# omerbt/TokenFlow

Hardware: NVIDIA H100
Metric: frames/sec for 40-frame 512x512 SD1.5 50-step edit (higher is better)
Workload: dtype fp16

## Files before the change

### tokenflow_b200/csrc/tf_common.cuh

```cuda
#pragma once

#include <cuda.h>
#include <cuda_fp16.h>
#include <cuda_runtime.h>
#include <stdint.h>
#include <stdio.h>

namespace tf {

void set_last_error(const char* fmt, ...);
int  check_cuda(cudaError_t e, const char* what);

enum Status : int {
  TF_OK = 0,
  TF_ERR_INVALID_ARGUMENT = 1,
  TF_ERR_CUDA = 2,
  TF_ERR_UNSUPPORTED = 3,
  TF_ERR_DRIVER = 4,
};

CUresult encode_tiled(CUtensorMap* map, CUtensorMapDataType dtype, uint32_t rank, const void* base,
                      const uint64_t* dims, const uint64_t* strides_bytes ,
                      const uint32_t* box, CUtensorMapSwizzle swizzle);

int sm_count();

#ifdef __CUDACC__
__device__ __forceinline__ uint32_t smem_u32(const void* p) {
  return static_cast<uint32_t>(__cvta_generic_to_shared(p));
}
__device__ __forceinline__ uint32_t lane_id() { return threadIdx.x & 31u; }

__device__ __forceinline__ void mbar_init(uint64_t* bar, uint32_t count) {
  asm volatile("mbarrier.init.shared::cta.b64 [%0], %1;" ::"r"(smem_u32(bar)), "r"(count) : "memory");
}
__device__ __forceinline__ void fence_mbar_init() {
  asm volatile("fence.mbarrier_init.release.cluster;" ::: "memory");
}
__device__ __forceinline__ void mbar_arrive(uint64_t* bar) {
  asm volatile("mbarrier.arrive.shared::cta.b64 _, [%0];" ::"r"(smem_u32(bar)) : "memory");
}
__device__ __forceinline__ void mbar_arrive_expect_tx(uint64_t* bar, uint32_t bytes) {
  asm volatile("mbarrier.arrive.expect_tx.shared::cta.b64 _, [%0], %1;" ::"r"(smem_u32(bar)), "r"(bytes)
               : "memory");
}
__device__ __forceinline__ bool mbar_try_wait(uint64_t* bar, uint32_t parity) {
  uint32_t ok;
  asm volatile(
      "{\n\t.reg .pred p;\n\t"
      "mbarrier.try_wait.parity.shared::cta.b64 p, [%1], %2;\n\t"
      "selp.u32 %0, 1, 0, p;\n\t}\n"
      : "=r"(ok)
      : "r"(smem_u32(bar)), "r"(parity)
      : "memory");
  return ok != 0;
}
__device__ __forceinline__ uint64_t global_timer_ns() {
  uint64_t t;
  asm volatile("mov.u64 %0, %%globaltimer;" : "=l"(t));
  return t;
}
__device__ __forceinline__ void mbar_wait(uint64_t* bar, uint32_t parity) {
  uint32_t spins = 0;
  uint64_t t0 = 0;
  while (!mbar_try_wait(bar, parity)) {
    if ((++spins & 2047u) == 0) {
      const uint64_t now = global_timer_ns();
      if (t0 == 0) t0 = now;
      if (now - t0 > 2000000000ull) __trap();
    }
  }
}

__device__ __forceinline__ void tma_prefetch_desc(const CUtensorMap* m) {
  asm volatile("prefetch.tensormap [%0];" ::"l"(reinterpret_cast<uint64_t>(m)) : "memory");
}
__device__ __forceinline__ void tma_load_3d(void* smem_dst, const CUtensorMap* m, uint64_t* bar, int c0,
                                            int c1, int c2) {
  asm volatile(
      "cp.async.bulk.tensor.3d.shared::cluster.global.tile.mbarrier::complete_tx::bytes"
      " [%0], [%1, {%3, %4, %5}], [%2];"
      ::"r"(smem_u32(smem_dst)), "l"(reinterpret_cast<uint64_t>(m)), "r"(smem_u32(bar)), "r"(c0), "r"(c1),
      "r"(c2)
      : "memory");
}
__device__ __forceinline__ void tma_load_4d(void* smem_dst, const CUtensorMap* m, uint64_t* bar, int c0,
                                            int c1, int c2, int c3) {
  asm volatile(
      "cp.async.bulk.tensor.4d.shared::cluster.global.tile.mbarrier::complete_tx::bytes"
      " [%0], [%1, {%3, %4, %5, %6}], [%2];"
      ::"r"(smem_u32(smem_dst)), "l"(reinterpret_cast<uint64_t>(m)), "r"(smem_u32(bar)), "r"(c0), "r"(c1),
      "r"(c2), "r"(c3)
      : "memory");
}

__device__ __forceinline__ uint64_t wgmma_desc(uint32_t smem_addr, uint32_t lbo_bytes, uint32_t sbo_bytes) {
  uint64_t d = 0;
  d |= static_cast<uint64_t>((smem_addr & 0x3FFFFu) >> 4);
  d |= static_cast<uint64_t>((lbo_bytes >> 4) & 0x3FFFu) << 16;
  d |= static_cast<uint64_t>((sbo_bytes >> 4) & 0x3FFFu) << 32;
  d |= static_cast<uint64_t>(1) << 62;
  return d;
}
__device__ __forceinline__ void wgmma_fence() { asm volatile("wgmma.fence.sync.aligned;" ::: "memory"); }
__device__ __forceinline__ void wgmma_commit() { asm volatile("wgmma.commit_group.sync.aligned;" ::: "memory"); }
template <int kPending>
__device__ __forceinline__ void wgmma_wait() {
  asm volatile("wgmma.wait_group.sync.aligned %0;" ::"n"(kPending) : "memory");
}
template <int N>
__device__ __forceinline__ void reg_fence(float (&r)[N]) {
#pragma unroll
  for (int i = 0; i < N; ++i) asm volatile("" : "+f"(r[i])::"memory");
}

__device__ __forceinline__ uint32_t pack_f16x2_rn(float lo, float hi) {
  uint32_t r;
  asm("cvt.rn.f16x2.f32 %0, %1, %2;" : "=r"(r) : "f"(hi), "f"(lo));
  return r;
}
__device__ __forceinline__ float fast_exp2(float x) {
  float y;
  asm("ex2.approx.ftz.f32 %0, %1;" : "=f"(y) : "f"(x));
  return y;
}
#endif

}
```

### tokenflow_b200/csrc/tf_ext_attn.cu

```cuda
#include <cmath>
#include <type_traits>

#include "tf_common.cuh"
#include "tf_kernels.h"
#include "tf_wgmma.cuh"

namespace tf {
namespace {

constexpr int kBlockM = 128;
constexpr int kMaxStages = 8;
constexpr int kSmemBudget = 227 * 1024;

struct AttnCtl {
  uint64_t q_full;
  uint64_t full[kMaxStages];
  uint64_t empty[kMaxStages];
};

struct AttnParams {
  int S, heads, d;
  int tiles_m;
  int stages;
  float scale_log2;
  long long out_tok_stride;
  int q_row0;
  int q_row_end;
  int out_rows;
};

struct Item {
  int out_u, out_c, q, k0, v_u0, v_c0, n_kv;
};
__device__ __forceinline__ Item item_of(const AttnTable& t, int i) {
  const AttnSample& s = t.s[i];
  return {s.out_sample, -1, s.q_sample, s.k_sample0, s.v_sample0, -1, s.n_kv};
}
__device__ __forceinline__ Item item_of(const AttnPairTable& t, int i) {
  const AttnPair& p = t.p[i];
  return {p.out_u, p.out_c, p.q_sample, p.k_sample0, p.v_u0, p.v_c0, p.n_kv};
}

template <int kDChunks, int kBlockN, int kNPV, class Tab>
__global__ void __launch_bounds__(256, 1)
ext_attn_kernel(const __grid_constant__ CUtensorMap map_q, const __grid_constant__ CUtensorMap map_k,
                const __grid_constant__ CUtensorMap map_v, const __grid_constant__ Tab tab, const AttnParams prm,
                __half* __restrict__ out) {
  constexpr int kNV = std::is_same<Tab, AttnPairTable>::value ? 2 : 1;
  constexpr int kQChunkBytes = kBlockM * 128;
  constexpr int kKVChunkBytes = kBlockN * 128;
  constexpr int kQBytes = kDChunks * kQChunkBytes;
  constexpr int kTileBytes = kDChunks * kKVChunkBytes;
  constexpr int kStageBytes = (1 + kNV) * kTileBytes;
  constexpr int kS = kBlockN / 2;
  constexpr int kO = kNPV / 2;
  static_assert(kNPV <= 64 * kDChunks, "P V width exceeds the loaded channels");

  extern __shared__ uint8_t smem_raw[];
  uint8_t* smem = reinterpret_cast<uint8_t*>((reinterpret_cast<uintptr_t>(smem_raw) + 1023) & ~uintptr_t(1023));
  uint8_t* q_smem = smem;
  uint8_t* ring = smem + kQBytes;
  AttnCtl* ctl = reinterpret_cast<AttnCtl*>(ring + prm.stages * kStageBytes);

  const int S = prm.S, d = prm.d, stages = prm.stages;
  const int per_sample = prm.heads * prm.tiles_m;
  const int slot = blockIdx.x / per_sample;
  const int rem = blockIdx.x - slot * per_sample;
  const int head = rem / prm.tiles_m;
  const int m0 = prm.q_row0 + (rem - head * prm.tiles_m) * kBlockM;
  const Item it = item_of(tab, slot);
  const int tiles_per_slab = (S + kBlockN - 1) / kBlockN;
  const int T = it.n_kv * tiles_per_slab;
  const int ksteps = (d + 15) / 16;

  auto load_tile = [&](int t) {
    const int st = t % stages;
    const int slab = t / tiles_per_slab;
    const int n0 = (t - slab * tiles_per_slab) * kBlockN;
    uint8_t* dst = ring + st * kStageBytes;
    mbar_arrive_expect_tx(&ctl->full[st], (uint32_t)kStageBytes);
#pragma unroll
    for (int c = 0; c < kDChunks; ++c) {
      tma_load_4d(dst + c * kKVChunkBytes, &map_k, &ctl->full[st], c * 64, head, n0, it.k0 + slab);
      tma_load_4d(dst + kTileBytes + c * kKVChunkBytes, &map_v, &ctl->full[st], c * 64, head, n0, it.v_u0 + slab);
      if (kNV == 2)
        tma_load_4d(dst + 2 * kTileBytes + c * kKVChunkBytes, &map_v, &ctl->full[st], c * 64, head, n0,
                    it.v_c0 + slab);
    }
  };

  if (threadIdx.x == 0) {
    tma_prefetch_desc(&map_q);
    tma_prefetch_desc(&map_k);
    tma_prefetch_desc(&map_v);
    mbar_init(&ctl->q_full, 1);
    for (int i = 0; i < stages; ++i) {
      mbar_init(&ctl->full[i], 1);
      mbar_init(&ctl->empty[i], 8);
    }
    fence_mbar_init();
  }
  __syncthreads();
  if (threadIdx.x == 0) {
    mbar_arrive_expect_tx(&ctl->q_full, (uint32_t)kQBytes);
#pragma unroll
    for (int c = 0; c < kDChunks; ++c) tma_load_4d(q_smem + c * kQChunkBytes, &map_q, &ctl->q_full, c * 64, head, m0, it.q);
    for (int t = 0; t < stages && t < T; ++t) load_tile(t);
  }
  __syncwarp();

  const int wg = threadIdx.x >> 7;
  const int lane = threadIdx.x & 31;
  const int wrow = ((threadIdx.x >> 5) & 3) * 16 + (lane >> 2);
  const int qcol = 2 * (lane & 3);

  float o[kNV][kO];
#pragma unroll
  for (int v = 0; v < kNV; ++v)
#pragma unroll
    for (int i = 0; i < kO; ++i) o[v][i] = 0.f;
  float m_r[2] = {-INFINITY, -INFINITY}, l_r[2] = {0.f, 0.f};
  const float sl2 = prm.scale_log2;

  const uint32_t q_addr = smem_u32(q_smem) + wg * 64 * 128;
  const uint32_t ring_addr = smem_u32(ring);
  mbar_wait(&ctl->q_full, 0);
  __syncwarp();

  for (int t = 0; t < T; ++t) {
    const int st = t % stages;
    mbar_wait(&ctl->full[st], (uint32_t)(t / stages) & 1u);
    __syncwarp();
    const uint32_t k_addr = ring_addr + st * kStageBytes;

    float s[kS];
    wgmma_fence();
    for (int kk = 0; kk < ksteps; ++kk) {
      const uint32_t off = (kk & 3) * 32;
      wgmma_ss<kBlockN>(s, wgmma_desc(q_addr + (kk >> 2) * kQChunkBytes + off, 16, 1024),
                        wgmma_desc(k_addr + (kk >> 2) * kKVChunkBytes + off, 16, 1024), kk > 0 ? 1u : 0u);
    }
    wgmma_commit();
    wgmma_wait<0>();
    reg_fence(s);

    const int n0 = (t % tiles_per_slab) * kBlockN;
    if (n0 + kBlockN > S) {
      const int valid = S - n0;
#pragma unroll
      for (int j = 0; j < kBlockN / 8; ++j) {
        const int c = 8 * j + qcol;
        if (c >= valid) { s[4 * j] = -INFINITY; s[4 * j + 2] = -INFINITY; }
        if (c + 1 >= valid) { s[4 * j + 1] = -INFINITY; s[4 * j + 3] = -INFINITY; }
      }
    }

    float mx[2] = {-INFINITY, -INFINITY};
#pragma unroll
    for (int j = 0; j < kBlockN / 8; ++j) {
      mx[0] = fmaxf(mx[0], fmaxf(s[4 * j], s[4 * j + 1]));
      mx[1] = fmaxf(mx[1], fmaxf(s[4 * j + 2], s[4 * j + 3]));
    }
    float corr[2], mneg[2];
#pragma unroll
    for (int r = 0; r < 2; ++r) {
      mx[r] = fmaxf(mx[r], __shfl_xor_sync(0xffffffffu, mx[r], 1));
      mx[r] = fmaxf(mx[r], __shfl_xor_sync(0xffffffffu, mx[r], 2));
      const float m_new = fmaxf(m_r[r], mx[r] * sl2);
      corr[r] = fast_exp2(m_r[r] - m_new);
      m_r[r] = m_new;
      mneg[r] = -m_new;
      l_r[r] *= corr[r];
    }
    uint32_t pa[kBlockN / 16][4];
#pragma unroll
    for (int j = 0; j < kBlockN / 8; ++j) {
      const float p0 = fast_exp2(fmaf(s[4 * j], sl2, mneg[0]));
      const float p1 = fast_exp2(fmaf(s[4 * j + 1], sl2, mneg[0]));
      const float p2 = fast_exp2(fmaf(s[4 * j + 2], sl2, mneg[1]));
      const float p3 = fast_exp2(fmaf(s[4 * j + 3], sl2, mneg[1]));
      l_r[0] += p0 + p1;
      l_r[1] += p2 + p3;
      pa[j >> 1][(j & 1) * 2 + 0] = pack_f16x2_rn(p0, p1);
      pa[j >> 1][(j & 1) * 2 + 1] = pack_f16x2_rn(p2, p3);
    }
#pragma unroll
    for (int v = 0; v < kNV; ++v)
#pragma unroll
      for (int j = 0; j < kO / 4; ++j) {
        o[v][4 * j] *= corr[0]; o[v][4 * j + 1] *= corr[0];
        o[v][4 * j + 2] *= corr[1]; o[v][4 * j + 3] *= corr[1];
      }

#pragma unroll
    for (int v = 0; v < kNV; ++v) reg_fence(o[v]);
    wgmma_fence();
#pragma unroll
    for (int kk = 0; kk < kBlockN / 16; ++kk)
#pragma unroll
      for (int v = 0; v < kNV; ++v)
        wgmma_rs<kNPV>(o[v], pa[kk], wgmma_desc(k_addr + (1 + v) * kTileBytes + kk * 16 * 128, kKVChunkBytes, 1024), 1u);
    wgmma_commit();
    wgmma_wait<0>();
#pragma unroll
    for (int v = 0; v < kNV; ++v) reg_fence(o[v]);

    __syncwarp();
    if (lane == 0) mbar_arrive(&ctl->empty[st]);
    if (threadIdx.x == 0 && t >= 1 && t - 1 + stages < T) {
      const int pt = t - 1;
      mbar_wait(&ctl->empty[pt % stages], (uint32_t)(pt / stages) & 1u);
      load_tile(pt + stages);
    }
    __syncwarp();
  }

#pragma unroll
  for (int r = 0; r < 2; ++r) {
    l_r[r] += __shfl_xor_sync(0xffffffffu, l_r[r], 1);
    l_r[r] += __shfl_xor_sync(0xffffffffu, l_r[r], 2);
    l_r[r] = 1.f / l_r[r];
  }
#pragma unroll
  for (int v = 0; v < kNV; ++v) {
    const int out_slab = v == 0 ? it.out_u : it.out_c;
#pragma unroll
    for (int r = 0; r < 2; ++r) {
      const int tok = m0 + wg * 64 + wrow + 8 * r;
      if (tok >= prm.q_row_end) continue;
      __half* dst = out + ((long long)out_slab * prm.out_rows + (tok - prm.q_row0)) * prm.out_tok_stride + head * d;
#pragma unroll
      for (int j = 0; j < kO / 4; ++j) {
        const int c = 8 * j + qcol;
        if (c < d)
          *reinterpret_cast<uint32_t*>(dst + c) = pack_f16x2_rn(o[v][4 * j + 2 * r] * l_r[r], o[v][4 * j + 2 * r + 1] * l_r[r]);
      }
    }
  }
}

template <int kDChunks, int kBlockN, int kNPV, class Tab>
int launch_cfg(const void* q, const void* k, const void* v, long long q_tok_stride, long long kv_tok_stride,
               int q_samples_total, int kv_samples_total, const Tab& tab, int n_items, int S, int heads, int d,
               float scale, void* out, int q_row0, int q_nrows, cudaStream_t stream) {
  constexpr int kNV = std::is_same<Tab, AttnPairTable>::value ? 2 : 1;
  constexpr int kQBytes = kDChunks * kBlockM * 128;
  constexpr int kStageBytes = (1 + kNV) * kDChunks * kBlockN * 128;
  int stages = (kSmemBudget - 2048 - kQBytes) / kStageBytes;
  if (stages > kMaxStages) stages = kMaxStages;
  if (stages < 2) { set_last_error("tf_ext_attn: configuration does not fit shared memory"); return TF_ERR_UNSUPPORTED; }
  const size_t smem_bytes = 1024 + kQBytes + (size_t)stages * kStageBytes + sizeof(AttnCtl);

  CUtensorMap map_q, map_k, map_v;
  auto make = [&](CUtensorMap* m, const void* base, long long tok_stride, int samples, int box_rows) -> int {
    const uint64_t dims[4] = {(uint64_t)d, (uint64_t)heads, (uint64_t)S, (uint64_t)samples};
    const uint64_t strides[3] = {(uint64_t)d * 2, (uint64_t)tok_stride * 2, (uint64_t)S * tok_stride * 2};
    const uint32_t box[4] = {64, 1, (uint32_t)box_rows, 1};
    CUresult r = encode_tiled(m, CU_TENSOR_MAP_DATA_TYPE_FLOAT16, 4, base, dims, strides, box,
                              CU_TENSOR_MAP_SWIZZLE_128B);
    if (r != CUDA_SUCCESS) { set_last_error("tf_ext_attn: cuTensorMapEncodeTiled failed: %d", (int)r); return TF_ERR_DRIVER; }
    return TF_OK;
  };
  if (int e = make(&map_q, q, q_tok_stride, q_samples_total, kBlockM)) return e;
  if (int e = make(&map_k, k, kv_tok_stride, kv_samples_total, kBlockN)) return e;
  if (int e = make(&map_v, v, kv_tok_stride, kv_samples_total, kBlockN)) return e;

  AttnParams prm;
  prm.S = S; prm.heads = heads; prm.d = d;
  prm.q_row0 = q_row0; prm.q_row_end = (q_row0 + q_nrows < S) ? q_row0 + q_nrows : S; prm.out_rows = q_nrows;
  prm.tiles_m = (prm.q_row_end - q_row0 + kBlockM - 1) / kBlockM;
  prm.stages = stages;
  prm.scale_log2 = scale * 1.4426950408889634f;
  prm.out_tok_stride = (long long)heads * d;

  auto kern = ext_attn_kernel<kDChunks, kBlockN, kNPV, Tab>;
  if (check_cuda(cudaFuncSetAttribute(kern, cudaFuncAttributeMaxDynamicSharedMemorySize, (int)smem_bytes),
                 "tf_ext_attn smem attribute"))
    return TF_ERR_CUDA;
  const long long grid = (long long)n_items * heads * prm.tiles_m;
  kern<<<(unsigned)grid, 256, smem_bytes, stream>>>(map_q, map_k, map_v, tab, prm, static_cast<__half*>(out));
  return check_cuda(cudaGetLastError(), "tf_ext_attn launch");
}

template <class Tab>
int dispatch(const void* q, const void* k, const void* v, long long q_tok_stride, long long kv_tok_stride,
             int q_samples_total, int kv_samples_total, const Tab& tab, int n_items, int S, int heads, int d,
             float scale, void* out, int q_row0, int q_nrows, cudaStream_t stream) {
  constexpr bool kPair = std::is_same<Tab, AttnPairTable>::value;
#define TF_CFG(C, N, P)                                                                                          \
  case P:                                                                                                       \
    if constexpr (!kPair || P <= 64)                                                                            \
      return launch_cfg<C, N, P, Tab>(q, k, v, q_tok_stride, kv_tok_stride, q_samples_total, kv_samples_total,  \
                                      tab, n_items, S, heads, d, scale, out, q_row0, q_nrows, stream);          \
    break
  switch ((d + 15) / 16 * 16) {
    TF_CFG(1, 128, 16); TF_CFG(1, 128, 32); TF_CFG(1, 128, 48); TF_CFG(1, 128, 64);
    TF_CFG(2, 128, 80); TF_CFG(2, 128, 96); TF_CFG(2, 128, 112); TF_CFG(2, 128, 128);
    TF_CFG(3, 64, 144); TF_CFG(3, 64, 160); TF_CFG(3, 64, 176); TF_CFG(3, 64, 192);
    default: break;
  }
#undef TF_CFG
  set_last_error("tf_ext_attn: head dim %d > 192 is not supported", d);
  return TF_ERR_UNSUPPORTED;
}

}

int launch_ext_attn(const void* q, const void* k, const void* v, long long q_tok_stride, long long kv_tok_stride,
                    int q_samples_total, int kv_samples_total, const AttnTable& tab, int n_out, int S, int heads,
                    int d, float scale, void* out, int q_row0, int q_nrows, cudaStream_t stream) {
  if (n_out == 0 || S == 0 || q_nrows <= 0 || q_row0 >= S) return TF_OK;
  return dispatch(q, k, v, q_tok_stride, kv_tok_stride, q_samples_total, kv_samples_total, tab, n_out, S, heads, d,
                  scale, out, q_row0, q_nrows, stream);
}

bool ext_attn_pairs_supported(int d) {
  return d <= 64;
}

int launch_ext_attn_pairs(const void* q, const void* k, const void* v, long long q_tok_stride, long long kv_tok_stride,
                          int q_samples_total, int kv_samples_total, const AttnPairTable& tab, int n_pairs, int S,
                          int heads, int d, float scale, void* out, int q_row0, int q_nrows, cudaStream_t stream) {
  if (n_pairs == 0 || S == 0 || q_nrows <= 0 || q_row0 >= S) return TF_OK;
  if (!ext_attn_pairs_supported(d)) {
    set_last_error("tf_ext_attn: paired kernel does not cover d=%d", d);
    return TF_ERR_UNSUPPORTED;
  }
  return dispatch(q, k, v, q_tok_stride, kv_tok_stride, q_samples_total, kv_samples_total, tab, n_pairs, S, heads, d,
                  scale, out, q_row0, q_nrows, stream);
}

}
```

Before: 2.886.

## Overlap QK and PV wgmma across iterations with ping-pong warpgroup scheduling

Restructures the extended-attention main loop so the QK^T wgmma for tile t is issued together with the PV wgmma for tile t-1, and softmax runs while PV is in flight. Named barriers make the two warpgroups take turns issuing tensor-core work, in the style of FlashAttention-3. The empty mbarriers are replaced by a shared atomic counter, and the last warp to release a stage issues its refill. This adds register pressure (s and pa are live across iterations) and more complex synchronization, which risks spills or ordering bugs in the barrier and atomic refill path.

```diff
diff --git a/tokenflow_b200/csrc/tf_common.cuh b/tokenflow_b200/csrc/tf_common.cuh
--- a/tokenflow_b200/csrc/tf_common.cuh
+++ b/tokenflow_b200/csrc/tf_common.cuh
@@ -72,6 +72,13 @@
   }
 }
 
+__device__ __forceinline__ void named_bar_sync(uint32_t id, uint32_t count) {
+  asm volatile("bar.sync %0, %1;" ::"r"(id), "r"(count) : "memory");
+}
+__device__ __forceinline__ void named_bar_arrive(uint32_t id, uint32_t count) {
+  asm volatile("bar.arrive %0, %1;" ::"r"(id), "r"(count) : "memory");
+}
+
 __device__ __forceinline__ void tma_prefetch_desc(const CUtensorMap* m) {
   asm volatile("prefetch.tensormap [%0];" ::"l"(reinterpret_cast<uint64_t>(m)) : "memory");
 }
diff --git a/tokenflow_b200/csrc/tf_ext_attn.cu b/tokenflow_b200/csrc/tf_ext_attn.cu
--- a/tokenflow_b200/csrc/tf_ext_attn.cu
+++ b/tokenflow_b200/csrc/tf_ext_attn.cu
@@ -15,7 +15,7 @@
 struct AttnCtl {
   uint64_t q_full;
   uint64_t full[kMaxStages];
-  uint64_t empty[kMaxStages];
+  uint32_t released[kMaxStages];
 };
 
 struct AttnParams {
@@ -41,8 +41,32 @@
   return {p.out_u, p.out_c, p.q_sample, p.k_sample0, p.v_u0, p.v_c0, p.n_kv};
 }
 
+constexpr int kThreads = 256;
+constexpr int kWarps = kThreads / 32;
+constexpr uint32_t kTurnBar = 1;
+
+template <int kBlockN, int kNPV, int kQChunkBytes, int kKVChunkBytes>
+__device__ __forceinline__ void issue_qk(float (&s)[kBlockN / 2], uint32_t q_addr, uint32_t k_addr) {
+#pragma unroll
+  for (int kk = 0; kk < kNPV / 16; ++kk) {
+    const uint32_t off = (kk & 3) * 32;
+    wgmma_ss<kBlockN>(s, wgmma_desc(q_addr + (kk >> 2) * kQChunkBytes + off, 16, 1024),
+                      wgmma_desc(k_addr + (kk >> 2) * kKVChunkBytes + off, 16, 1024), kk > 0 ? 1u : 0u);
+  }
+}
+
+template <int kBlockN, int kNPV, int kNV, int kTileBytes, int kKVChunkBytes>
+__device__ __forceinline__ void issue_pv(float (&o)[kNV][kNPV / 2], const uint32_t (&pa)[kBlockN / 16][4],
+                                         uint32_t k_addr) {
+#pragma unroll
+  for (int kk = 0; kk < kBlockN / 16; ++kk)
+#pragma unroll
+    for (int v = 0; v < kNV; ++v)
+      wgmma_rs<kNPV>(o[v], pa[kk], wgmma_desc(k_addr + (1 + v) * kTileBytes + kk * 16 * 128, kKVChunkBytes, 1024), 1u);
+}
+
 template <int kDChunks, int kBlockN, int kNPV, class Tab>
-__global__ void __launch_bounds__(256, 1)
+__global__ void __launch_bounds__(kThreads, 1)
 ext_attn_kernel(const __grid_constant__ CUtensorMap map_q, const __grid_constant__ CUtensorMap map_k,
                 const __grid_constant__ CUtensorMap map_v, const __grid_constant__ Tab tab, const AttnParams prm,
                 __half* __restrict__ out) {
@@ -71,20 +95,19 @@
   const Item it = item_of(tab, slot);
   const int tiles_per_slab = (S + kBlockN - 1) / kBlockN;
   const int T = it.n_kv * tiles_per_slab;
-  const int ksteps = (d + 15) / 16;
 
   auto load_tile = [&](int t) {
-    const int st = t % stages;
+    const int stage = t % stages;
     const int slab = t / tiles_per_slab;
-    const int n0 = (t - slab * tiles_per_slab) * kBlockN;
-    uint8_t* dst = ring + st * kStageBytes;
-    mbar_arrive_expect_tx(&ctl->full[st], (uint32_t)kStageBytes);
+    const int kn0 = (t - slab * tiles_per_slab) * kBlockN;
+    uint8_t* dst = ring + stage * kStageBytes;
+    mbar_arrive_expect_tx(&ctl->full[stage], (uint32_t)kStageBytes);
 #pragma unroll
     for (int c = 0; c < kDChunks; ++c) {
-      tma_load_4d(dst + c * kKVChunkBytes, &map_k, &ctl->full[st], c * 64, head, n0, it.k0 + slab);
-      tma_load_4d(dst + kTileBytes + c * kKVChunkBytes, &map_v, &ctl->full[st], c * 64, head, n0, it.v_u0 + slab);
+      tma_load_4d(dst + c * kKVChunkBytes, &map_k, &ctl->full[stage], c * 64, head, kn0, it.k0 + slab);
+      tma_load_4d(dst + kTileBytes + c * kKVChunkBytes, &map_v, &ctl->full[stage], c * 64, head, kn0, it.v_u0 + slab);
       if (kNV == 2)
-        tma_load_4d(dst + 2 * kTileBytes + c * kKVChunkBytes, &map_v, &ctl->full[st], c * 64, head, n0,
+        tma_load_4d(dst + 2 * kTileBytes + c * kKVChunkBytes, &map_v, &ctl->full[stage], c * 64, head, kn0,
                     it.v_c0 + slab);
     }
   };
@@ -96,7 +119,7 @@
     mbar_init(&ctl->q_full, 1);
     for (int i = 0; i < stages; ++i) {
       mbar_init(&ctl->full[i], 1);
-      mbar_init(&ctl->empty[i], 8);
+      ctl->released[i] = 0;
     }
     fence_mbar_init();
   }
@@ -104,15 +127,16 @@
   if (threadIdx.x == 0) {
     mbar_arrive_expect_tx(&ctl->q_full, (uint32_t)kQBytes);
 #pragma unroll
-    for (int c = 0; c < kDChunks; ++c) tma_load_4d(q_smem + c * kQChunkBytes, &map_q, &ctl->q_full, c * 64, head, m0, it.q);
+    for (int c = 0; c < kDChunks; ++c)
+      tma_load_4d(q_smem + c * kQChunkBytes, &map_q, &ctl->q_full, c * 64, head, m0, it.q);
     for (int t = 0; t < stages && t < T; ++t) load_tile(t);
   }
-  __syncwarp();
-
-  const int wg = threadIdx.x >> 7;
+
+  const int cw = threadIdx.x >> 7;
   const int lane = threadIdx.x & 31;
   const int wrow = ((threadIdx.x >> 5) & 3) * 16 + (lane >> 2);
   const int qcol = 2 * (lane & 3);
+  const uint32_t my_turn = kTurnBar + cw, other_turn = kTurnBar + (cw ^ 1);
 
   float o[kNV][kO];
 #pragma unroll
@@ -122,29 +146,40 @@
   float m_r[2] = {-INFINITY, -INFINITY}, l_r[2] = {0.f, 0.f};
   const float sl2 = prm.scale_log2;
 
-  const uint32_t q_addr = smem_u32(q_smem) + wg * 64 * 128;
+  const uint32_t q_addr = smem_u32(q_smem) + cw * 64 * 128;
   const uint32_t ring_addr = smem_u32(ring);
+  int st = 0, n0 = 0;
+  uint32_t ph = 0;
+  auto advance = [&]() {
+    if (++st == stages) { st = 0; ph ^= 1u; }
+    n0 += kBlockN;
+    if (n0 >= S) n0 = 0;
+  };
+  auto stage_addr = [&](int stage) { return ring_addr + stage * kStageBytes; };
+  auto wait_full = [&]() {
+    mbar_wait(&ctl->full[st], ph);
+    __syncwarp();
+  };
+  auto release = [&](int stage, int t) {
+    __syncwarp();
+    if (lane == 0) {
+      __threadfence_block();
+      if (atomicAdd(&ctl->released[stage], 1u) == kWarps - 1) {
+        __threadfence_block();
+        ctl->released[stage] = 0;
+        if (t + stages < T) load_tile(t + stages);
+      }
+    }
+  };
+
+  if (cw == 1) named_bar_arrive(kTurnBar, kThreads);
   mbar_wait(&ctl->q_full, 0);
   __syncwarp();
 
-  for (int t = 0; t < T; ++t) {
-    const int st = t % stages;
-    mbar_wait(&ctl->full[st], (uint32_t)(t / stages) & 1u);
-    __syncwarp();
-    const uint32_t k_addr = ring_addr + st * kStageBytes;
-
-    float s[kS];
-    wgmma_fence();
-    for (int kk = 0; kk < ksteps; ++kk) {
-      const uint32_t off = (kk & 3) * 32;
-      wgmma_ss<kBlockN>(s, wgmma_desc(q_addr + (kk >> 2) * kQChunkBytes + off, 16, 1024),
-                        wgmma_desc(k_addr + (kk >> 2) * kKVChunkBytes + off, 16, 1024), kk > 0 ? 1u : 0u);
-    }
-    wgmma_commit();
-    wgmma_wait<0>();
-    reg_fence(s);
-
-    const int n0 = (t % tiles_per_slab) * kBlockN;
+  float s[kS];
+  uint32_t pa[kBlockN / 16][4];
+
+  auto softmax = [&](float (&corr)[2]) {
     if (n0 + kBlockN > S) {
       const int valid = S - n0;
 #pragma unroll
@@ -154,14 +189,13 @@
         if (c + 1 >= valid) { s[4 * j + 1] = -INFINITY; s[4 * j + 3] = -INFINITY; }
       }
     }
-
     float mx[2] = {-INFINITY, -INFINITY};
 #pragma unroll
     for (int j = 0; j < kBlockN / 8; ++j) {
       mx[0] = fmaxf(mx[0], fmaxf(s[4 * j], s[4 * j + 1]));
       mx[1] = fmaxf(mx[1], fmaxf(s[4 * j + 2], s[4 * j + 3]));
     }
-    float corr[2], mneg[2];
+    float mneg[2];
 #pragma unroll
     for (int r = 0; r < 2; ++r) {
       mx[r] = fmaxf(mx[r], __shfl_xor_sync(0xffffffffu, mx[r], 1));
@@ -172,7 +206,6 @@
       mneg[r] = -m_new;
       l_r[r] *= corr[r];
     }
-    uint32_t pa[kBlockN / 16][4];
 #pragma unroll
     for (int j = 0; j < kBlockN / 8; ++j) {
       const float p0 = fast_exp2(fmaf(s[4 * j], sl2, mneg[0]));
@@ -181,9 +214,10 @@
       const float p3 = fast_exp2(fmaf(s[4 * j + 3], sl2, mneg[1]));
       l_r[0] += p0 + p1;
       l_r[1] += p2 + p3;
-      pa[j >> 1][(j & 1) * 2 + 0] = pack_f16x2_rn(p0, p1);
-      pa[j >> 1][(j & 1) * 2 + 1] = pack_f16x2_rn(p2, p3);
-    }
+      s[4 * j] = p0; s[4 * j + 1] = p1; s[4 * j + 2] = p2; s[4 * j + 3] = p3;
+    }
+  };
+  auto rescale_and_pack = [&](const float (&corr)[2]) {
 #pragma unroll
     for (int v = 0; v < kNV; ++v)
 #pragma unroll
@@ -191,28 +225,63 @@
         o[v][4 * j] *= corr[0]; o[v][4 * j + 1] *= corr[0];
         o[v][4 * j + 2] *= corr[1]; o[v][4 * j + 3] *= corr[1];
       }
-
+#pragma unroll
+    for (int j = 0; j < kBlockN / 8; ++j) {
+      pa[j >> 1][(j & 1) * 2 + 0] = pack_f16x2_rn(s[4 * j], s[4 * j + 1]);
+      pa[j >> 1][(j & 1) * 2 + 1] = pack_f16x2_rn(s[4 * j + 2], s[4 * j + 3]);
+    }
+  };
+
+  {
+    wait_full();
+    named_bar_sync(my_turn, kThreads);
+    wgmma_fence();
+    issue_qk<kBlockN, kNPV, kQChunkBytes, kKVChunkBytes>(s, q_addr, stage_addr(st));
+    wgmma_commit();
+    named_bar_arrive(other_turn, kThreads);
+    wgmma_wait<0>();
+    reg_fence(s);
+    float corr[2];
+    softmax(corr);
+    rescale_and_pack(corr);
+  }
+  int st_prev = st;
+  advance();
+  for (int t = 1; t < T; ++t) {
+    wait_full();
+    named_bar_sync(my_turn, kThreads);
 #pragma unroll
     for (int v = 0; v < kNV; ++v) reg_fence(o[v]);
     wgmma_fence();
-#pragma unroll
-    for (int kk = 0; kk < kBlockN / 16; ++kk)
-#pragma unroll
-      for (int v = 0; v < kNV; ++v)
-        wgmma_rs<kNPV>(o[v], pa[kk], wgmma_desc(k_addr + (1 + v) * kTileBytes + kk * 16 * 128, kKVChunkBytes, 1024), 1u);
+    issue_qk<kBlockN, kNPV, kQChunkBytes, kKVChunkBytes>(s, q_addr, stage_addr(st));
     wgmma_commit();
+    issue_pv<kBlockN, kNPV, kNV, kTileBytes, kKVChunkBytes>(o, pa, stage_addr(st_prev));
+    wgmma_commit();
+    named_bar_arrive(other_turn, kThreads);
+    wgmma_wait<1>();
+    reg_fence(s);
+    float corr[2];
+    softmax(corr);
     wgmma_wait<0>();
 #pragma unroll
     for (int v = 0; v < kNV; ++v) reg_fence(o[v]);
-
-    __syncwarp();
-    if (lane == 0) mbar_arrive(&ctl->empty[st]);
-    if (threadIdx.x == 0 && t >= 1 && t - 1 + stages < T) {
-      const int pt = t - 1;
-      mbar_wait(&ctl->empty[pt % stages], (uint32_t)(pt / stages) & 1u);
-      load_tile(pt + stages);
-    }
-    __syncwarp();
+    release(st_prev, t - 1);
+    rescale_and_pack(corr);
+    st_prev = st;
+    advance();
+  }
+  {
+    named_bar_sync(my_turn, kThreads);
+#pragma unroll
+    for (int v = 0; v < kNV; ++v) reg_fence(o[v]);
+    wgmma_fence();
+    issue_pv<kBlockN, kNPV, kNV, kTileBytes, kKVChunkBytes>(o, pa, stage_addr(st_prev));
+    wgmma_commit();
+    if (cw == 0) named_bar_arrive(other_turn, kThreads);
+    wgmma_wait<0>();
+#pragma unroll
+    for (int v = 0; v < kNV; ++v) reg_fence(o[v]);
+    release(st_prev, T - 1);
   }
 
 #pragma unroll
@@ -226,7 +295,7 @@
     const int out_slab = v == 0 ? it.out_u : it.out_c;
 #pragma unroll
     for (int r = 0; r < 2; ++r) {
-      const int tok = m0 + wg * 64 + wrow + 8 * r;
+      const int tok = m0 + cw * 64 + wrow + 8 * r;
       if (tok >= prm.q_row_end) continue;
       __half* dst = out + ((long long)out_slab * prm.out_rows + (tok - prm.q_row0)) * prm.out_tok_stride + head * d;
 #pragma unroll
@@ -278,7 +347,7 @@
                  "tf_ext_attn smem attribute"))
     return TF_ERR_CUDA;
   const long long grid = (long long)n_items * heads * prm.tiles_m;
-  kern<<<(unsigned)grid, 256, smem_bytes, stream>>>(map_q, map_k, map_v, tab, prm, static_cast<__half*>(out));
+  kern<<<(unsigned)grid, kThreads, smem_bytes, stream>>>(map_q, map_k, map_v, tab, prm, static_cast<__half*>(out));
   return check_cuda(cudaGetLastError(), "tf_ext_attn launch");
 }
 
```

Measured after the change: 2.917 (median of 6 runs). 1.01x the previous value.
